# slp-rl/slamkit

Measured on NVIDIA H100. Metric: speech-tokens/sec (SLAM seq=1024), higher is better.
Workload: dtype bf16

## Files before the change

### slamkit_b200/csrc/gemm_tcgen05.cu

```cuda
#include "common.cuh"
#include <cudaTypedefs.h>
#include <stdio.h>
#include <mutex>
#include <type_traits>
#include <string.h>
#include <stdlib.h>
#include "kernels.h"
#include "../../include/slamkit_b200.h"

namespace {

constexpr int BM = 128;
constexpr int BK = 64;
constexpr int MMA_K = 16;
constexpr int GEMM_THREADS = 288;


struct GemmParams {
  int M, N, K;
  int batch;
  int a_mode;
  int passes;
  void* C;
  void* C_lo;
  int ldc;
  const void* bias;
  int bias_f32;
  const bf16* residual;
  const bf16* residual_lo;
  int ldr;
  int tiles_m, tiles_n;
  int out_f32;
  int round_before_res;
  int act;
  int col_gin, col_gout;
  int splits;
  float* splitk_ws;
  int tma_store;
  int reg_epi;
  int pdl;
  int sk_units;
  int sk_groups;
  int sk_G;
  int sk_colunits;
  int sk_carry;
  int units, n_groups;
  float* sk_ws;
  uint32_t* sk_flags;
  int epi;
  const bf16* aux;
  int ld_aux;
  const bf16* rope_cos;
  const bf16* rope_sin;
  const int* rope_pos;
  int rope_T, rope_cols, rope_maxpos, rope_rot;
};

template <int BN, int EW = 4>
struct GemmCfg {
  static constexpr int A_BYTES = BM * BK * 2;
  static constexpr int B_ATOMS = (BN + 63) / 64;
  static constexpr int B_BYTES = B_ATOMS * 64 * BK * 2;
  static constexpr int STAGE_BYTES = A_BYTES + B_BYTES;
  static constexpr int STAGES = (BN > 128) ? 4 : (BN > 64 ? 6 : 8);
  static constexpr int STAGING_BYTES = 4 * 2 * 4096;
  static constexpr int BAR_BYTES = 256;
  static constexpr int SMEM_BYTES = STAGES * STAGE_BYTES + STAGING_BYTES + BAR_BYTES + 1024;
  static_assert(BN % 64 == 0 || (BN == 224 && EW == 4), "a 32-column tail chunk only on the 224-wide tile");
  static_assert(STAGES * STAGE_BYTES >= BM * BN * 4, "the parked fp32 accumulator must fit in the stage ring");
  static_assert(SMEM_BYTES <= 227 * 1024, "sm_90 allows 227 KB of shared memory per block");
};

template <int BN>
SK_DEVINL uint32_t acc_chunk_addr(uint32_t base, int row, int chunk) {
  return base + (uint32_t)row * (BN * 4) + (uint32_t)((chunk ^ (row & 7)) << 4);
}
template <int BN>
SK_DEVINL void acc_park(uint32_t base, const float (&d)[BN / 2], int wg, int warp_in_wg, int lane) {
  const int r0 = 64 * wg + 16 * warp_in_wg + (lane >> 2);
#pragma unroll
  for (int j = 0; j < BN / 8; ++j) {
    const int chunk = 2 * j + ((lane & 3) >> 1);
    const uint32_t off = (uint32_t)(lane & 1) * 8u;
    asm volatile("st.shared.v2.f32 [%0], {%1, %2};" ::"r"(acc_chunk_addr<BN>(base, r0, chunk) + off), "f"(d[4 * j]),
                 "f"(d[4 * j + 1]) : "memory");
    asm volatile("st.shared.v2.f32 [%0], {%1, %2};" ::"r"(acc_chunk_addr<BN>(base, r0 + 8, chunk) + off), "f"(d[4 * j + 2]),
                 "f"(d[4 * j + 3]) : "memory");
  }
}
template <int BN>
SK_DEVINL void acc_ld_32x32(uint32_t base, uint32_t ta, uint32_t (&r)[32]) {
  const int row = (int)(ta >> 16) + (int)(threadIdx.x & 31);
  const int c0 = (int)(ta & 0xffffu) >> 2;
#pragma unroll
  for (int i = 0; i < 8; ++i)
    asm volatile("ld.shared.v4.b32 {%0, %1, %2, %3}, [%4];"
                 : "=r"(r[4 * i]), "=r"(r[4 * i + 1]), "=r"(r[4 * i + 2]), "=r"(r[4 * i + 3])
                 : "r"(acc_chunk_addr<BN>(base, row, c0 + i)) : "memory");
}

SK_DEVINL uint32_t staging_addr(uint32_t sbuf, int lane, int j, bool tail) {
  return tail ? sbuf + (uint32_t)lane * 64u + (uint32_t)((j ^ ((lane >> 1) & 3)) << 4)
              : sbuf + (uint32_t)lane * 128u + (uint32_t)((j ^ (lane & 7)) << 4);
}

SK_DEVINL float gelu_erf(float y) {
  const float a = fabsf(y);
  float t;
  asm("rcp.approx.ftz.f32 %0, %1;" : "=f"(t) : "f"(fmaf(0.3275911f * 0.70710678118654752440f, a, 1.0f)));
  float s = fmaf(0.5f * 1.061405429f, t, 0.5f * -1.453152027f);
  s = fmaf(s, t, 0.5f * 1.421413741f);
  s = fmaf(s, t, 0.5f * -0.284496736f);
  s = fmaf(s, t, 0.5f * 0.254829592f);
  const float e = ex2_approx((y * y) * -0.72134752044448170368f);
  return fmaf(-a, (s * t) * e, fmaxf(y, 0.0f));
}

SK_DEVINL float gelu_exact(float x) { return x * 0.5f * (1.0f + erff(x * 0.70710678118654752440f)); }
SK_DEVINL float gelu_exact_grad(float x) {
  const float cdf = 0.5f * (1.0f + erff(x * 0.70710678118654752440f));
  const float pdf = expf(-0.5f * x * x) * 0.39894228040143267794f;
  return cdf + x * pdf;
}

SK_DEVINL void stmatrix_x4(uint32_t addr, uint32_t a, uint32_t b, uint32_t c, uint32_t d) {
  asm volatile("stmatrix.sync.aligned.m8n8.x4.shared.b16 [%0], {%1, %2, %3, %4};" ::"r"(addr), "r"(a), "r"(b), "r"(c),
               "r"(d) : "memory");
}

template <bool SK>
struct WorkIter {
  int num_kb, splits, kb_per_split, total_items, tiles_n;
  int G, colunits, carry, units, n_groups, sk_groups, grp, mem;
  long sk_total, sk_cur, sk_end;
  int next_unit, next_item;
  int tile, split, kb_begin, kb_end, role;
  long unit_end_it;
  SK_DEVINL WorkIter(const GemmParams& p, int num_kb_, int kb_per_split_, int total_items_) {
    num_kb = num_kb_;
    splits = p.splits;
    kb_per_split = kb_per_split_;
    total_items = total_items_;
    tiles_n = p.tiles_n;
    G = p.sk_G;
    colunits = p.sk_colunits;
    carry = p.sk_carry;
    units = p.units;
    n_groups = p.n_groups;
    sk_groups = p.sk_groups;
    tile = split = kb_begin = kb_end = role = 0;
    unit_end_it = 0;
    sk_total = sk_cur = sk_end = 0;
    next_item = (int)blockIdx.x;
    next_unit = 0;
    grp = mem = 0;
    if (SK && p.sk_units > 0) {
      grp = (int)blockIdx.x / G;
      mem = (int)blockIdx.x - grp * G;
      next_item = total_items;
      next_unit = grp < n_groups ? p.sk_units + grp : units;
      if (grp < sk_groups) {
        sk_total = (long)p.sk_units * num_kb;
        sk_cur = sk_total * grp / sk_groups;
        sk_end = sk_total * (grp + 1) / sk_groups;
      }
    }
  }
  SK_DEVINL int tile_of(int unit) const { return colunits ? mem * tiles_n + unit : unit * G + mem; }
  SK_DEVINL bool next() {
    if (SK && sk_cur < sk_end && carry) {
      const int unit = (int)((sk_end - 1) / num_kb);
      const long ustart = (long)unit * num_kb;
      const long b = sk_cur > ustart ? sk_cur : ustart;
      kb_begin = (int)(b - ustart);
      kb_end = (int)(sk_end - ustart);
// ... 86 lines not shown
    const uint32_t aw[4] = {av.x, av.y, av.z, av.w};
#pragma unroll
    for (int i = 0; i < 4; ++i) {
      const float2 f = unpack_bf16(aw[i]);
      v[2 * i] = bf16_round(bf16_round(v[2 * i]) + f.x);
      v[2 * i + 1] = bf16_round(bf16_round(v[2 * i + 1]) + f.y);
    }
  }
  if (!p.residual) return;
  const uint4 rv = *reinterpret_cast<const uint4*>(p.residual + row * p.ldr + ocol);
  const uint32_t rw[4] = {rv.x, rv.y, rv.z, rv.w};
#pragma unroll
  for (int i = 0; i < 4; ++i) {
    const float2 f = unpack_bf16(rw[i]);
    if (p.round_before_res) {
      v[2 * i] = bf16_round(v[2 * i]) + f.x;
      v[2 * i + 1] = bf16_round(v[2 * i + 1]) + f.y;
    } else {
      v[2 * i] += f.x;
      v[2 * i + 1] += f.y;
    }
  }
  if (p.residual_lo) {
    const uint4 lv = *reinterpret_cast<const uint4*>(p.residual_lo + row * p.ldr + ocol);
    const uint32_t lw[4] = {lv.x, lv.y, lv.z, lv.w};
#pragma unroll
    for (int i = 0; i < 4; ++i) {
      const float2 f = unpack_bf16(lw[i]);
      v[2 * i] += f.x;
      v[2 * i + 1] += f.y;
    }
  }
}

constexpr int SK_SLOT_FLOATS = BM * 256;
SK_DEVINL size_t sk_slot_off(int chunk, int j4, int row_in_tile) { return ((size_t)(chunk * 8 + j4) * BM + row_in_tile) * 4; }

SK_DEVINL void sk_fixup_add(uint32_t (&r)[32], const float* ws, int chunk, int row_in_tile, int first_cta, int G, int n) {
  for (int c0 = 0; c0 < n; ++c0) {
    const float* slot = ws + (size_t)(first_cta + c0 * G) * SK_SLOT_FLOATS;
    float4 a[8];
#pragma unroll
    for (int j = 0; j < 8; ++j) a[j] = __ldcg(reinterpret_cast<const float4*>(slot + sk_slot_off(chunk, j, row_in_tile)));
#pragma unroll
    for (int j = 0; j < 8; ++j) {
      r[4 * j + 0] = __float_as_uint(__uint_as_float(r[4 * j + 0]) + a[j].x);
      r[4 * j + 1] = __float_as_uint(__uint_as_float(r[4 * j + 1]) + a[j].y);
      r[4 * j + 2] = __float_as_uint(__uint_as_float(r[4 * j + 2]) + a[j].z);
      r[4 * j + 3] = __float_as_uint(__uint_as_float(r[4 * j + 3]) + a[j].w);
    }
  }
}

template <int BN, bool A_MN, bool B_MN, bool SK, int EW>
__global__ void __launch_bounds__(GEMM_THREADS, 1)
gemm_wgmma_kernel(const __grid_constant__ CUtensorMap tmA, const __grid_constant__ CUtensorMap tmB,
                  const __grid_constant__ CUtensorMap tmA_lo, const __grid_constant__ CUtensorMap tmB_lo,
                  const __grid_constant__ CUtensorMap tmC, const __grid_constant__ CUtensorMap tmAux, GemmParams p) {
  using Cfg = GemmCfg<BN, EW>;
  static_assert(EW == 4 || (EW == 8 && BN == 256 && !SK), "8 epilogue warps: plain 256-wide tiles only");
  constexpr int CS = EW / 4;
  constexpr int NC64 = BN / 64;
  constexpr bool TAIL = BN % 64 != 0;
  griddep_launch();
  extern __shared__ uint8_t smem_raw[];
  const uint32_t smem_base = (smem_u32(smem_raw) + 1023u) & ~1023u;
  const uint32_t staging_base = smem_base + Cfg::STAGES * Cfg::STAGE_BYTES;
  const uint32_t bar_base = staging_base + Cfg::STAGING_BYTES;
  auto full_bar = [&](int s) { return bar_base + 8u * s; };
  auto empty_bar = [&](int s) { return bar_base + 8u * (Cfg::STAGES + s); };
  const uint32_t acc_free = bar_base + 8u * (2 * Cfg::STAGES);

  const int warp = threadIdx.x >> 5;
  const int lane = threadIdx.x & 31;
  const int tiles_per_batch = p.tiles_m * p.tiles_n;
  const int total_items = tiles_per_batch * p.batch * p.splits;
  const int num_kb_total = (p.K + BK - 1) / BK;
  const int kb_per_split = (num_kb_total + p.splits - 1) / p.splits;
  constexpr uint32_t STAGE_TX = Cfg::A_BYTES + (B_MN ? Cfg::B_ATOMS * 64 * BK * 2 : BN * BK * 2);

  if (threadIdx.x == 0) {
    tma_prefetch_desc(&tmA);
    tma_prefetch_desc(&tmB);
    for (int s = 0; s < Cfg::STAGES; ++s) {
      mbar_init(full_bar(s), 1);
      mbar_init(empty_bar(s), 8);
    }
    mbar_init(acc_free, 1);
    fence_mbar_init();
  }
  __syncthreads();
  griddep_wait();

  if (warp == 8) {
    if (lane == 0) {
      const bool split = p.passes == 3;
      const int n_stage = split ? Cfg::STAGES / 2 : Cfg::STAGES;
      const uint32_t stage_bytes = split ? 2u * Cfg::STAGE_BYTES : (uint32_t)Cfg::STAGE_BYTES;
      int stage = 0;
      uint32_t phase = 0;
      uint32_t acc_phase = 0;
      bool first = true;
      WorkIter<SK> w(p, num_kb_total, kb_per_split, total_items);
      while (w.next()) {
        if (!first && !p.reg_epi) {
          mbar_wait_nocall(acc_free, acc_phase);
          acc_phase ^= 1u;
        }
        first = false;
        const int bidx = w.tile / tiles_per_batch;
        const int r = w.tile - bidx * tiles_per_batch;
        const int m0 = (r / p.tiles_n) * BM;
        const int n_blk = r % p.tiles_n;
        const int n0 = n_blk * BN;
        for (int kb = w.kb_begin; kb < w.kb_end; ++kb) {
          mbar_wait_nocall(empty_bar(stage), phase ^ 1u);
          const uint32_t fb = full_bar(stage);
          mbar_arrive_expect_tx(fb, split ? 2u * STAGE_TX : STAGE_TX);
          for (int part = 0; part < (split ? 2 : 1); ++part) {
            const CUtensorMap* mapA = part ? &tmA_lo : &tmA;
            const CUtensorMap* mapB = part ? &tmB_lo : &tmB;
            const uint32_t sA = smem_base + stage * stage_bytes + part * Cfg::STAGE_BYTES;
            const uint32_t sB = sA + Cfg::A_BYTES;
            if (!A_MN) {
              if (p.a_mode & 2) {
                if (p.a_mode & 1) tma_load_3d(sA, mapA, fb, n_blk * 64, m0 + kb, bidx);
                else tma_load_3d(sA, mapA, fb, kb * BK, m0, bidx);
              } else {
                tma_load_2d(sA, mapA, fb, kb * BK, m0);
              }
            } else {
#pragma unroll
              for (int j = 0; j < BM / 64; ++j) tma_load_2d(sA + j * (BK * 128), mapA, fb, m0 + 64 * j, kb * BK);
            }
            if (!B_MN) {
              tma_load_2d(sB, mapB, fb, kb * BK, n0);
            } else {
#pragma unroll
              for (int j = 0; j < Cfg::B_ATOMS; ++j) tma_load_2d(sB + j * (BK * 128), mapB, fb, n0 + 64 * j, kb * BK);
            }
          }
          if (++stage == n_stage) { stage = 0; phase ^= 1u; }
        }
      }
    }
  } else {
    const int wg = warp >> 2;
    const int q = warp & 3;
    const int chalf = warp >> 2;
    const bool epi_warp = warp < EW;
    auto acc_ld = [&](uint32_t ta, uint32_t (&r)[32]) { acc_ld_32x32<BN>(smem_base, ta, r); };
    const bool split = p.passes == 3;
    const int n_stage = split ? Cfg::STAGES / 2 : Cfg::STAGES;
    const uint32_t stage_bytes = split ? 2u * Cfg::STAGE_BYTES : (uint32_t)Cfg::STAGE_BYTES;
    int stage = 0;
    uint32_t phase = 0;
    uint32_t store_cnt = 0;
    auto release_acc = [&] {
      fence_proxy_async();
      named_bar_sync(1, 256);
      if (threadIdx.x == 0) mbar_arrive(acc_free);
    };
    WorkIter<SK> w(p, num_kb_total, kb_per_split, total_items);
    while (w.next()) {
      {
        auto reg_epilogue = [&](const float (&acc)[BN / 2]) {
          const int rr = w.tile;
          const int m0 = (rr / p.tiles_n) * BM, n0 = (rr % p.tiles_n) * BN;
          const int row0 = m0 + 16 * warp;
          const uint32_t stg = staging_base + (uint32_t)warp * 4096u;
          auto emit = [&](const uint32_t (&pk)[16], const CUtensorMap* map, int col, bool tail) {
            const uint32_t sbuf = stg + (store_cnt & 1u) * 2048u;
            if (lane == 0) tma_store_wait_read<1>();
            __syncwarp();
            const int srow = (lane & 7) + (lane & 8);
#pragma unroll
            for (int jj = 0; jj < (tail ? 4 : 8); jj += 2) {
              const int ch = jj + (lane >> 4);
              const uint32_t addr = tail ? sbuf + (uint32_t)srow * 64u + (uint32_t)((ch ^ ((srow >> 1) & 3)) << 4)
                                         : sbuf + (uint32_t)srow * 128u + (uint32_t)((ch ^ (srow & 7)) << 4);
              stmatrix_x4(addr, pk[2 * jj], pk[2 * jj + 1], pk[2 * jj + 2], pk[2 * jj + 3]);
            }
            fence_proxy_async();
            __syncwarp();
            if (lane == 0) {
              tma_store_2d(map, sbuf, col, row0);
              tma_store_commit();
            }
            ++store_cnt;
          };
          auto pair_bf16 = [&](int j, int h) { return pack_bf16(acc[4 * j + 2 * h], acc[4 * j + 2 * h + 1]); };
          if (p.epi == 1) {
            if constexpr (BN == 256) {
#pragma unroll
              for (int i = 0; i < 2; ++i) {
                uint32_t pk[16];
#pragma unroll
                for (int t = 0; t < 16; ++t) pk[t] = pair_bf16(8 * i + (t >> 1), t & 1);
                emit(pk, &tmC, n0 + 64 * i, false);
#pragma unroll
                for (int t = 0; t < 16; ++t) pk[t] = pair_bf16(16 + 8 * i + (t >> 1), t & 1);
                emit(pk, &tmC, n0 + 128 + 64 * i, false);
#pragma unroll
                for (int t = 0; t < 16; ++t) {
                  const float2 gf = unpack_bf16(pair_bf16(8 * i + (t >> 1), t & 1));
                  const float2 uf = unpack_bf16(pair_bf16(16 + 8 * i + (t >> 1), t & 1));
                  const float2 sb = unpack_bf16(pack_bf16(silu_f(gf.x), silu_f(gf.y)));
                  pk[t] = pack_bf16(sb.x * uf.x, sb.y * uf.y);
                }
                emit(pk, &tmAux, (n0 >> 1) + 64 * i, false);
              }
            }
          } else {
#pragma unroll
            for (int c2 = 0; c2 < (BN + 63) / 64; ++c2) {
              const bool tail = BN % 64 != 0 && c2 == BN / 64;
              if (n0 + 64 * c2 >= p.N) continue;
              uint32_t pk[16];
#pragma unroll
              for (int t = 0; t < (tail ? 8 : 16); ++t) pk[t] = pair_bf16(8 * c2 + (t >> 1), t & 1);
              emit(pk, tail ? &tmAux : &tmC, n0 + 64 * c2, tail);
            }
          }
        };
        auto mainloop_park = [&](float (&acc)[BN / 2]) {
          const int k_iters = max(0, w.kb_end - w.kb_begin);
          int prev = -1;
          for (int kb = 0; kb < k_iters; ++kb) {
            mbar_wait_nocall(full_bar(stage), phase);
            wgmma_fence();
            const uint32_t s_hi = smem_base + stage * stage_bytes;
            for (int g = 0; g < (split ? 3 : 1); ++g) {
              const uint32_t sA = s_hi + (g == 2 ? Cfg::STAGE_BYTES : 0) + (uint32_t)wg * 8192u;
              const uint32_t sB = s_hi + Cfg::A_BYTES + (g == 1 ? Cfg::STAGE_BYTES : 0);
#pragma unroll
              for (int k = 0; k < BK / MMA_K; ++k) {
                const uint64_t adesc = A_MN ? gmma_desc_sw128(sA + k * (MMA_K * 128), BK * 128, 1024)
                                            : gmma_desc_sw128(sA + k * (MMA_K * 2), 16, 1024);
                const uint64_t bdesc = B_MN ? gmma_desc_sw128(sB + k * (MMA_K * 128), BK * 128, 1024)
                                            : gmma_desc_sw128(sB + k * (MMA_K * 2), 16, 1024);
                wgmma_bf16<BN, A_MN ? 1 : 0, B_MN ? 1 : 0>(acc, adesc, bdesc);
              }
            }
            wgmma_commit();
            wgmma_wait<1>();
            if (prev >= 0 && lane == 0) mbar_arrive(empty_bar(prev));
            prev = stage;
            if (++stage == n_stage) { stage = 0; phase ^= 1u; }
          }
          wgmma_wait<0>();
          if (prev >= 0 && lane == 0) mbar_arrive(empty_bar(prev));
          if constexpr (!SK && EW == 4) {
            if (p.reg_epi) {
              reg_epilogue(acc);
              return;
            }
          }
          named_bar_sync(1, 256);
          acc_park<BN>(smem_base, acc, wg, warp & 3, lane);
          named_bar_sync(1, 256);
        };
        if (SK && w.role == 3) {
          float acc[BN / 2];
          const int src = (int)blockIdx.x - w.G;
          if (threadIdx.x == 0) {
            for (int qq = 0; qq < 4; ++qq) {
              const uint32_t* f = p.sk_flags + src * 4 + qq;
              const uint64_t t0 = globaltimer_ns();
              while (ld_acquire_u32(f) == 0u) {
                __nanosleep(64);
                if (globaltimer_ns() - t0 > 8000000000ull) __trap();
              }
            }
            for (int qq = 0; qq < 4; ++qq) p.sk_flags[src * 4 + qq] = 0u;
          }
          named_bar_sync(1, 256);
          const float* slot = p.sk_ws + (size_t)src * SK_SLOT_FLOATS;
          const int r0 = 64 * wg + 16 * (warp & 3) + (lane >> 2);
#pragma unroll
          for (int j = 0; j < BN / 8; ++j) {
            const int col = 8 * j + 2 * (lane & 3);
#pragma unroll
            for (int h = 0; h < 2; ++h) {
              const float2 v = __ldcg(reinterpret_cast<const float2*>(slot + sk_slot_off(col >> 5, (col & 31) >> 2, r0 + 8 * h) +
                                                                      (col & 3)));
              acc[4 * j + 2 * h] = v.x;
              acc[4 * j + 2 * h + 1] = v.y;
            }
          }
          mainloop_park(acc);
        } else {
          float acc[BN / 2];
#pragma unroll
          for (int i = 0; i < BN / 2; ++i) acc[i] = 0.f;
          mainloop_park(acc);
        }
      }
      if (!SK && p.reg_epi) continue;
      if (!epi_warp) {
        release_acc();
        continue;
      }
      const int split_idx = w.split;
      const int bidx = w.tile / tiles_per_batch;
      const int rr = w.tile - bidx * tiles_per_batch;
      const int m0 = (rr / p.tiles_n) * BM;
      const int n0 = (rr % p.tiles_n) * BN;
      if (!SK && p.tma_store && p.epi == 2) {
        const int lpiece = lane & 7, lrsub = lane >> 3;
        const uint32_t sX = staging_base + (uint32_t)warp * (EW == 4 ? 8192u : 4096u);
        constexpr int NCH = BN / 64 / CS;
        const int c_lo = chalf * NCH;
        auto piece_off = [&](int bidx, int m0, int n0, int c2, size_t ld) -> size_t {
          const int acol = n0 + c2 * 64;
          const int gcol = (acol >> 7) * 256 + (acol & 127) + lpiece * 8;
          return (((size_t)bidx * p.M + m0 + q * 32 + lrsub) * ld + gcol) * sizeof(bf16);
        };
        const size_t row4_in = (size_t)4 * p.ld_aux * sizeof(bf16), row4_out = (size_t)4 * p.ldc * sizeof(bf16);
        uint4 gv[8], uv[8];
        auto gu_load_k = [&](int k, const uint8_t* base, int m0, int n0, int c2) {
          const int rin = m0 + q * 32 + 4 * k + lrsub;
          if (rin < p.M && n0 + c2 * 64 < p.N) {
            gv[k] = ldg128(base + k * row4_in);
            uv[k] = ldg128(base + k * row4_in + 256);
          } else {
            gv[k] = make_uint4(0u, 0u, 0u, 0u);
            uv[k] = make_uint4(0u, 0u, 0u, 0u);
          }
        };
        {
          const uint8_t* base = reinterpret_cast<const uint8_t*>(p.aux) + piece_off(bidx, m0, n0, c_lo, (size_t)p.ld_aux);
#pragma unroll
          for (int k = 0; k < 8; ++k) gu_load_k(k, base, m0, n0, c_lo);
        }
        const uint32_t taddr = (uint32_t)(q * 32) << 16;
#pragma unroll 1
        for (int c2 = c_lo; c2 < c_lo + NCH; ++c2) {
          const bool col_ok = n0 + c2 * 64 < p.N;
          {
            uint32_t r0[32], r1[32];
            acc_ld(taddr + c2 * 64, r0);
            acc_ld(taddr + c2 * 64 + 32, r1);
#pragma unroll
            for (int j = 0; j < 8; ++j) {
              const uint32_t* r = j < 4 ? r0 + 8 * j : r1 + 8 * (j - 4);
              const uint32_t dst = sX + (uint32_t)lane * 128u + (uint32_t)((j ^ (lane & 7)) << 4);
              asm volatile("st.shared.v4.b32 [%0], {%1, %2, %3, %4};" ::"r"(dst),
                           "r"(pack_bf16(__uint_as_float(r[0]), __uint_as_float(r[1]))),
                           "r"(pack_bf16(__uint_as_float(r[2]), __uint_as_float(r[3]))),
                           "r"(pack_bf16(__uint_as_float(r[4]), __uint_as_float(r[5]))),
                           "r"(pack_bf16(__uint_as_float(r[6]), __uint_as_float(r[7])))
                           : "memory");
            }
          }
          __syncwarp();
          const bool refill = c2 + 1 < c_lo + NCH;
          const int fm0 = m0, fn0 = n0, fc2 = c2 + 1;
          const uint8_t* fbase = reinterpret_cast<const uint8_t*>(p.aux) + piece_off(bidx, fm0, fn0, fc2, (size_t)p.ld_aux);
          uint8_t* obase = reinterpret_cast<uint8_t*>(p.C) + piece_off(bidx, m0, n0, c2, (size_t)p.ldc);
#pragma unroll
          for (int k = 0; k < 8; ++k) {
            const int rr2 = 4 * k + lrsub;
            const uint32_t off = (uint32_t)rr2 * 128u + (uint32_t)((lpiece ^ (rr2 & 7)) << 4);
            uint32_t dw[4];
            asm volatile("ld.shared.v4.b32 {%0, %1, %2, %3}, [%4];" : "=r"(dw[0]), "=r"(dw[1]), "=r"(dw[2]), "=r"(dw[3]) : "r"(sX + off));
            const uint32_t gw[4] = {gv[k].x, gv[k].y, gv[k].z, gv[k].w}, uw[4] = {uv[k].x, uv[k].y, uv[k].z, uv[k].w};
            if (refill) gu_load_k(k, fbase, fm0, fn0, fc2);
            uint32_t og[4], ou[4];
#pragma unroll
            for (int e = 0; e < 4; ++e) {
              const float2 gf = unpack_bf16(gw[e]);
              const float s0 = sigmoid_f(gf.x), s1 = sigmoid_f(gf.y);
              const uint32_t sil2 = pack_bf16(gf.x * s0, gf.y * s1);
              const float ds0 = s0 * (1.0f + gf.x * (1.0f - s0)), ds1 = s1 * (1.0f + gf.y * (1.0f - s1));
              const bf162 d2 = *reinterpret_cast<const bf162*>(&dw[e]);
              bf162 du2 = __hmul2(d2, *reinterpret_cast<const bf162*>(&uw[e]));
              bf162 o2 = __hmul2(d2, *reinterpret_cast<const bf162*>(&sil2));
              const float2 duf = __bfloat1622float2(du2);
              og[e] = pack_bf16(duf.x * ds0, duf.y * ds1);
              ou[e] = *reinterpret_cast<uint32_t*>(&o2);
            }
            if (col_ok && m0 + q * 32 + rr2 < p.M) {
              stg128(obase + k * row4_out, make_uint4(og[0], og[1], og[2], og[3]));
              stg128(obase + k * row4_out + 256, make_uint4(ou[0], ou[1], ou[2], ou[3]));
            }
          }
          __syncwarp();
        }
        release_acc();
        continue;
      }
      const int row_in_tile = q * 32 + lane;
      const int row_in = m0 + row_in_tile;
      const bool row_ok = row_in < p.M;
      const size_t row = (size_t)bidx * p.M + row_in;
      const uint32_t taddr = (uint32_t)(q * 32) << 16;
      const int first_contrib = (int)blockIdx.x + w.G;
      const int n_contrib = (SK && w.role == 2) ? w.n_contrib() : 0;
      if (SK && w.role == 1) {
        float* slot = p.sk_ws + (size_t)blockIdx.x * SK_SLOT_FLOATS;
#pragma unroll 1
        for (int c = 0; c < BN / 32; ++c) {
          uint32_t r[32];
          acc_ld(taddr + c * 32, r);
#pragma unroll
          for (int j = 0; j < 8; ++j)
            __stcg(reinterpret_cast<float4*>(slot + sk_slot_off(c, j, row_in_tile)),
                   make_float4(__uint_as_float(r[4 * j]), __uint_as_float(r[4 * j + 1]), __uint_as_float(r[4 * j + 2]),
                               __uint_as_float(r[4 * j + 3])));
        }
        __threadfence();
        __syncwarp();
        if (lane == 0) st_release_u32(p.sk_flags + blockIdx.x * 4 + q, 1u);
      } else {
        if (SK && w.role == 2) {
          if (lane == 0) {
            for (int i = 0; i < n_contrib; ++i) {
              const int c = first_contrib + i * w.G;
              const uint32_t* f = p.sk_flags + c * 4 + q;
              const uint64_t t0 = globaltimer_ns();
              while (ld_acquire_u32(f) == 0u) {
                __nanosleep(64);
                if (globaltimer_ns() - t0 > 8000000000ull) __trap();
              }
            }
          }
          __syncwarp();
        }
        auto stage_store = [&](const CUtensorMap* map, const uint32_t (&pk)[32], int col, auto tail_c) {
          constexpr bool tail = decltype(tail_c)::value;
          const uint32_t sbuf = staging_base + (EW == 4 ? (uint32_t)warp * 8192u + (store_cnt & 1u) * 4096u : (uint32_t)warp * 4096u);
          if (lane == 0) {
            if constexpr (EW == 4) tma_store_wait_read<1>(); else tma_store_wait_read<0>();
          }
// ... 427 lines not shown
PFN_cuTensorMapEncodeTiled_v12000 g_encode = nullptr;
std::once_flag g_encode_once;

void load_encode() {
  void* fn = nullptr;
  cudaDriverEntryPointQueryResult qres;
  cudaError_t e = cudaGetDriverEntryPoint("cuTensorMapEncodeTiled", &fn, cudaEnableDefault, &qres);
  if (e == cudaSuccess && qres == cudaDriverEntryPointSuccess) g_encode = (PFN_cuTensorMapEncodeTiled_v12000)fn;
}

}

int sk_make_tmap_2d(CUtensorMap* out, const void* ptr, int elem_bytes, uint64_t inner, uint64_t outer, uint64_t ld,
                    uint32_t box_inner, uint32_t box_outer) {
  std::call_once(g_encode_once, load_encode);
  SK_REQUIRE(g_encode != nullptr, "cuTensorMapEncodeTiled driver entry point not available");
  SK_REQUIRE((reinterpret_cast<uintptr_t>(ptr) & 15) == 0, "TMA base pointer must be 16-byte aligned");
  SK_REQUIRE((ld * elem_bytes) % 16 == 0, "TMA row pitch must be a multiple of 16 bytes (ld=%llu)",
             (unsigned long long)ld);
  SK_REQUIRE(box_inner * elem_bytes == 128 || box_inner * elem_bytes == 64, "box inner extent must be 128 (or 64) bytes");
  cuuint64_t dims[2] = {inner, outer};
  cuuint64_t strides[1] = {ld * (uint64_t)elem_bytes};
  cuuint32_t box[2] = {box_inner, box_outer};
  cuuint32_t estr[2] = {1, 1};
  CUtensorMapDataType dt = elem_bytes == 2 ? CU_TENSOR_MAP_DATA_TYPE_BFLOAT16 : CU_TENSOR_MAP_DATA_TYPE_FLOAT32;
  CUresult r = g_encode(out, dt, 2, const_cast<void*>(ptr), dims, strides, box, estr, CU_TENSOR_MAP_INTERLEAVE_NONE,
                        box_inner * elem_bytes == 64 ? CU_TENSOR_MAP_SWIZZLE_64B : CU_TENSOR_MAP_SWIZZLE_128B,
                        CU_TENSOR_MAP_L2_PROMOTION_L2_256B,
                        CU_TENSOR_MAP_FLOAT_OOB_FILL_NONE);
  SK_REQUIRE(r == CUDA_SUCCESS, "cuTensorMapEncodeTiled failed with CUresult %d (inner=%llu outer=%llu ld=%llu)", (int)r,
             (unsigned long long)inner, (unsigned long long)outer, (unsigned long long)ld);
  return 0;
}

int sk_make_tmap_3d(CUtensorMap* out, const void* ptr, uint64_t inner, uint64_t rows, uint64_t batch, uint64_t row_stride,
                    uint64_t batch_stride, uint32_t box_rows) {
  std::call_once(g_encode_once, load_encode);
  SK_REQUIRE(g_encode != nullptr, "cuTensorMapEncodeTiled driver entry point not available");
  SK_REQUIRE((reinterpret_cast<uintptr_t>(ptr) & 15) == 0, "TMA base pointer must be 16-byte aligned");
  SK_REQUIRE((row_stride * 2) % 16 == 0 && (batch_stride * 2) % 16 == 0, "TMA strides must be multiples of 16 bytes");
  cuuint64_t dims[3] = {inner, rows, batch};
  cuuint64_t strides[2] = {row_stride * 2, batch_stride * 2};
  cuuint32_t box[3] = {64, box_rows, 1};
  cuuint32_t estr[3] = {1, 1, 1};
  CUresult r = g_encode(out, CU_TENSOR_MAP_DATA_TYPE_BFLOAT16, 3, const_cast<void*>(ptr), dims, strides, box, estr,
                        CU_TENSOR_MAP_INTERLEAVE_NONE, CU_TENSOR_MAP_SWIZZLE_128B, CU_TENSOR_MAP_L2_PROMOTION_L2_256B,
                        CU_TENSOR_MAP_FLOAT_OOB_FILL_NONE);
  SK_REQUIRE(r == CUDA_SUCCESS, "cuTensorMapEncodeTiled(3d) failed with CUresult %d", (int)r);
  return 0;
}

namespace {

template <int BN, bool A_MN, bool B_MN, bool SK, int EW = 4>
int launch_gemm(const CUtensorMap* tm, const GemmParams& p, int grid, cudaStream_t stream) {
  using Cfg = GemmCfg<BN, EW>;
  static bool attr_set = false;
  if (!attr_set) {
    SK_CUDA_CHECK(cudaFuncSetAttribute(gemm_wgmma_kernel<BN, A_MN, B_MN, SK, EW>, cudaFuncAttributeMaxDynamicSharedMemorySize,
                                       Cfg::SMEM_BYTES));
    attr_set = true;
  }
  sk_prof_begin(0, stream);
  cudaError_t lerr = sk_launch_pdl_if(p.pdl != 0, gemm_wgmma_kernel<BN, A_MN, B_MN, SK, EW>, dim3(grid), dim3(GEMM_THREADS), (size_t)Cfg::SMEM_BYTES, stream,
                                   tm[0], tm[1], tm[2], tm[3], tm[4], tm[5], p);
  sk_prof_end(stream);
  SK_CUDA_CHECK(lerr);
  SK_LAUNCH_CHECK();
  return 0;
}

template <int BN, bool SK, int EW = 4>
int dispatch_major(bool a_mn, bool b_mn, const CUtensorMap* tm, const GemmParams& p, int grid, cudaStream_t s) {
  if (!a_mn && !b_mn) return launch_gemm<BN, false, false, SK, EW>(tm, p, grid, s);
  if (!a_mn && b_mn) return launch_gemm<BN, false, true, SK, EW>(tm, p, grid, s);
  if (a_mn && !b_mn) return launch_gemm<BN, true, false, SK, EW>(tm, p, grid, s);
  return launch_gemm<BN, true, true, SK, EW>(tm, p, grid, s);
}

inline int tile_cost(int bn) { return bn >= 256 ? 100 : (bn > 128 ? 61 + (bn - 128) * 39 / 128 : (bn == 128 ? 61 : 54)); }

constexpr size_t SK_FLAG_BYTES = 4096;

}

size_t sk_gemm_ws_min_bytes(void) { return (size_t)sk_num_sms() * SK_SLOT_FLOATS * sizeof(float) + SK_FLAG_BYTES; }

int sk_pick_bn(int M, int N, int force_bn, bool fit_forced, bool fit, bool whole_heads) {
  if (force_bn == 64 || force_bn == 128 || force_bn == 256) return force_bn;
  if (fit_forced && (force_bn == 192 || (force_bn == 224 && !whole_heads))) return force_bn;
  const int nsm = sk_num_sms();
  auto cost = [&](int bn) {
    const long tiles = (long)((M + BM - 1) / BM) * ((N + bn - 1) / bn);
    return ((tiles + nsm - 1) / nsm) * tile_cost(bn);
  };
  int best = 256;
  long best_cost = cost(256);
  for (const int bn : {128, 64}) {
    if (cost(bn) * 100 < best_cost * 75) {
      best_cost = cost(bn);
      best = bn;
    }
  }
  if (best == 256 && fit && N % 256 != 0) {
    for (const int bn : {224, 192}) {
      if (!(whole_heads && bn % 64 != 0) && cost(bn) * 100 < best_cost * 95) {
        best_cost = cost(bn);
        best = bn;
      }
    }
  }
  return best;
}

namespace {

int plan_gemm(const SkGemmEx& g, GemmParams& p, int& BN, int& ew, int& grid) {
// ... 95 lines not shown
      SK_REQUIRE(BN == 256 && g.N % 256 == 0 && g.aux_out && g.ld_aux_out % 8 == 0 && !g.bias,
                 "gemm: SwiGLU-forward epilogue needs N = 2F with F %% 128 == 0 and an act output");
    } else if (g.epi == 2) {
      SK_REQUIRE(BN == 256 && g.N % 128 == 0 && g.aux && g.ld_aux % 8 == 0 && !g.bias,
                 "gemm: SwiGLU-backward epilogue needs N = F with F %% 128 == 0 and the saved gu activation");
    } else if (g.epi == 3) {
      SK_REQUIRE(g.rope_cos && g.rope_sin && g.rope_T > 0 && g.rope_maxpos > 0 && g.rope_cols % 64 == 0 && g.N % 64 == 0 &&
                     !g.bias_f32,
                 "gemm: RoPE epilogue needs cos/sin tables, 64-column heads and a bf16 bias");
      SK_REQUIRE(p.rope_rot == 16 || p.rope_rot == 32 || p.rope_rot == 64,
                 "gemm: RoPE epilogue rotary width rope_rot=%d is not supported (16, 32 or 64)", g.rope_rot);
    } else if (g.epi == 4) {
      SK_REQUIRE(BN % 64 == 0 && g.N % 64 == 0 && g.aux_out && g.ld_aux_out >= g.N && g.ld_aux_out % 8 == 0 && !g.bias_f32 &&
                     (reinterpret_cast<uintptr_t>(g.aux_out) & 15) == 0,
                 "gemm: GELU-forward epilogue needs N %% 64 == 0, an act output (pitch >= N) and a bf16 bias");
    } else if (g.epi == 5) {
      SK_REQUIRE(BN % 64 == 0 && g.N % 64 == 0 && g.aux && g.ld_aux >= g.N && g.ld_aux % 8 == 0 && !g.bias &&
                     (reinterpret_cast<uintptr_t>(g.aux) & 15) == 0,
                 "gemm: GELU-backward epilogue needs N %% 64 == 0, the saved pre-activation (pitch >= N) and no bias");
    } else {
      SK_REQUIRE(false, "gemm: unknown fused epilogue %d", g.epi);
    }
  }
  p.sk_G = 1;
  if (sk_ok && BN == 256 && p.splits == 1 && num_kb >= sk_min_kb && (p.tiles_n <= 8 || p.tiles_m <= 8)) {
    const int colunits = p.tiles_n <= 8 ? 0 : 1;
    const int G = colunits ? p.tiles_m : p.tiles_n;
    const int units = colunits ? p.tiles_n : p.tiles_m;
    const int n_groups = nsm / G;
    const int rem = units % n_groups;
    const long slots = ((long)(units + n_groups - 1) / n_groups) * n_groups;
    const bool multiwave = units > n_groups;
    if (n_groups >= 1 && rem != 0 && (slots - units) * 100 >= slots * sk_min_idle &&
        (!colunits || multiwave || sk_env >= 2)) {
      if (colunits && multiwave) {
        p.sk_units = rem + n_groups;
        p.sk_groups = n_groups;
        p.sk_carry = 1;
      } else {
        p.sk_units = rem;
        p.sk_groups = n_groups < rem * sk_ranges ? n_groups : rem * sk_ranges;
      }
      p.sk_G = G;
      p.sk_colunits = colunits;
      p.units = units;
      p.n_groups = n_groups;
      p.sk_ws = reinterpret_cast<float*>(g.splitk_ws);
      p.sk_flags = reinterpret_cast<uint32_t*>(reinterpret_cast<uint8_t*>(g.splitk_ws) + ws_data_bytes);
    }
  }
  const long work = tiles * p.splits;
  grid = p.sk_units > 0 ? p.n_groups * p.sk_G : (int)(work < nsm ? work : nsm);
  static const int ew_env = [] { const char* e = getenv("SK_GEMM_EW"); return e ? atoi(e) : 0; }();
  ew = (p.sk_units == 0 && BN == 256 && p.tma_store && (ew_env == 8 || (ew_env == 0 && (g.epi == 2 || g.epi == 3 || g.epi == 4 || g.epi == 5)))) ? 8 : 4;
  p.reg_epi = (p.tma_store && p.sk_units == 0 && ew == 4 && !g.bias && !g.act && !g.residual && (g.epi == 0 || g.epi == 1)) ? 1 : 0;
  return 0;
}

}

int sk_gemm_plan_ex(const SkGemmEx& g, SkGemmPlan* out) {
  GemmParams p;
  int BN = 0, ew = 0, grid = 0;
  const int rc = plan_gemm(g, p, BN, ew, grid);
  if (rc) return rc;
  out->bn = BN;
  out->epi_warps = ew;
  out->splits = p.splits;
  out->sk_units = p.sk_units;
  out->sk_groups = p.sk_groups;
  out->sk_G = p.sk_G;
  out->sk_colunits = p.sk_colunits;
  out->tma_store = p.tma_store;
  out->grid = grid;
  return 0;
}

int sk_gemm_ex_launch(const SkGemmEx& g, cudaStream_t stream) {
  GemmParams p;
  int BN = 0, ew = 0, grid = 0;
  const int rc0 = plan_gemm(g, p, BN, ew, grid);
  if (rc0) return rc0;
  const bool use3d = g.a_rows > 0;
  CUtensorMap tm[6];
  const void* As[2] = {g.A, g.passes == 3 ? g.A_lo : g.A};
  const void* Bs[2] = {g.B, g.passes == 3 ? g.B_lo : g.B};
  for (int i = 0; i < 2; ++i) {
    int rc;
    CUtensorMap* ta = &tm[i == 0 ? 0 : 2];
    CUtensorMap* tb = &tm[i == 0 ? 1 : 3];
    if (use3d) {
      rc = sk_make_tmap_3d(ta, As[i], (uint64_t)g.a_inner, (uint64_t)g.a_rows, (uint64_t)g.batch, (uint64_t)g.a_row_stride,
                           (uint64_t)g.a_batch_stride, BM);
    } else if (!g.a_mn) {
      rc = sk_make_tmap_2d(ta, As[i], 2, (uint64_t)g.K, (uint64_t)g.M, (uint64_t)g.lda, BK, BM);
    } else {
      rc = sk_make_tmap_2d(ta, As[i], 2, (uint64_t)g.M, (uint64_t)g.K, (uint64_t)g.lda, 64, BK);
    }
    if (rc) return rc;
    if (!g.b_mn) rc = sk_make_tmap_2d(tb, Bs[i], 2, (uint64_t)g.K, (uint64_t)g.N, (uint64_t)g.ldb, BK, (uint32_t)BN);
    else         rc = sk_make_tmap_2d(tb, Bs[i], 2, (uint64_t)g.N, (uint64_t)g.K, (uint64_t)g.ldb, 64, BK);
    if (rc) return rc;
  }
  tm[4] = tm[0];
  const uint32_t box_rows = p.reg_epi ? 16 : 32;
  if (p.tma_store) {
    const int rc2 = sk_make_tmap_2d(&tm[4], g.C, 2, (uint64_t)(g.epi == 2 ? 2 * g.N : g.N), (uint64_t)g.M, (uint64_t)g.ldc, 64, box_rows);
    if (rc2) return rc2;
  }
  tm[5] = tm[4];
  if (g.epi == 1) {
    const int rc3 = sk_make_tmap_2d(&tm[5], g.aux_out, 2, (uint64_t)g.N / 2, (uint64_t)g.M, (uint64_t)g.ld_aux_out, 64, box_rows);
    if (rc3) return rc3;
  } else if (g.epi == 4) {
    const int rc3 = sk_make_tmap_2d(&tm[5], g.aux_out, 2, (uint64_t)g.N, (uint64_t)g.M, (uint64_t)g.ld_aux_out, 64, 32);
    if (rc3) return rc3;
  } else if (p.tma_store && BN % 64 != 0) {
    const int rc3 = sk_make_tmap_2d(&tm[5], g.C, 2, (uint64_t)g.N, (uint64_t)g.M, (uint64_t)g.ldc, 32, box_rows);
    if (rc3) return rc3;
  }
  int rc;
  if (p.sk_units > 0) {
    rc = dispatch_major<256, true>(g.a_mn, g.b_mn, tm, p, grid, stream);
  } else if (ew == 8) {
    rc = dispatch_major<256, false, 8>(g.a_mn, g.b_mn, tm, p, grid, stream);
  } else {
    switch (BN) {
      case 256: rc = dispatch_major<256, false>(g.a_mn, g.b_mn, tm, p, grid, stream); break;
      case 224: rc = dispatch_major<224, false>(g.a_mn, g.b_mn, tm, p, grid, stream); break;
      case 192: rc = dispatch_major<192, false>(g.a_mn, g.b_mn, tm, p, grid, stream); break;
      case 128: rc = dispatch_major<128, false>(g.a_mn, g.b_mn, tm, p, grid, stream); break;
      default:  rc = dispatch_major<64, false>(g.a_mn, g.b_mn, tm, p, grid, stream); break;
    }
  }
  if (rc) return rc;
  if (p.splits > 1) {
    SK_REQUIRE(g.residual == nullptr || g.residual == g.C, "gemm: split-K supports only in-place accumulation");
    const long n8 = (long)g.M * g.N / 8;
    int blocks = (int)((n8 + 255) / 256);
    if (blocks > sk_num_sms() * 8) blocks = sk_num_sms() * 8;
    sk_prof_begin(0, stream);
    SK_CUDA_CHECK(sk_launch_pdl(splitk_reduce_kernel, dim3(blocks), dim3(256), (size_t)(0), stream, p.splitk_ws, reinterpret_cast<bf16*>(g.C), g.M, g.N, g.ldc, p.splits,
                                                     g.residual != nullptr, g.round_before_res));
    sk_prof_end(stream);
    SK_LAUNCH_CHECK();
  }
  return 0;
}

SkGemmEx sk_gemm_desc(int M, int N, int K, const void* A, int lda, int a_mn, const void* B, int ldb, int b_mn, void* C,
                      int ldc, int out_f32, const void* bias, const void* residual, int ldr, int round_before_res, int act,
                      int force_bn, void* splitk_ws, size_t splitk_ws_bytes) {
  SkGemmEx g;
  memset(&g, 0, sizeof(g));
  g.M = M; g.N = N; g.K = K; g.batch = 1; g.passes = 1;
  g.A = A; g.lda = lda; g.a_mn = a_mn;
  g.B = B; g.ldb = ldb; g.b_mn = b_mn;
  g.C = C; g.ldc = ldc; g.out_f32 = out_f32;
  g.bias = bias; g.residual = residual; g.ldr = ldr; g.round_before_res = round_before_res; g.act = act;
  g.force_bn = force_bn;
  g.pdl = 1;
  g.splitk_ws = splitk_ws;
  g.splitk_ws_bytes = splitk_ws_bytes;
  return g;
}
int sk_gemm_launch(int M, int N, int K, const void* A, int lda, int a_mn, const void* B, int ldb, int b_mn, void* C,
                   int ldc, int out_f32, const void* bias, const void* residual, int ldr, int round_before_res, int act,
                   int force_bn, cudaStream_t stream, void* splitk_ws, size_t splitk_ws_bytes) {
  return sk_gemm_ex_launch(sk_gemm_desc(M, N, K, A, lda, a_mn, B, ldb, b_mn, C, ldc, out_f32, bias, residual, ldr,
                                        round_before_res, act, force_bn, splitk_ws, splitk_ws_bytes),
                           stream);
}

int sk_linear_swiglu_fwd_launch(int M, int F, int K, const void* x, const void* Wgu, void* gu, void* act, cudaStream_t s) {
  SkGemmEx g;
// ... 61 lines not shown
```

Baseline: 165,800.

## Fuse SwiGLU backward into register epilogue with TMA-prefetched gate/up operands

Adds a GU kernel variant for the epi==2 (SwiGLU backward) GEMM. The accumulator is combined in registers with gate/up operands that TMA double-buffers into per-warp shared memory, and the results go out through TMA stores, replacing the parked-accumulator shared-memory epilogue. It also adds a register epilogue with residual add for narrower tiles, and stops epi==2 from using 8 epilogue warps. The GU variant drops to 3 pipeline stages to make room for operand buffers, which may reduce mainloop latency hiding.

```diff
diff --git a/slamkit_b200/csrc/gemm_tcgen05.cu b/slamkit_b200/csrc/gemm_tcgen05.cu
--- a/slamkit_b200/csrc/gemm_tcgen05.cu
+++ b/slamkit_b200/csrc/gemm_tcgen05.cu
@@ -56,16 +56,17 @@
   int rope_T, rope_cols, rope_maxpos, rope_rot;
 };
 
-template <int BN, int EW = 4>
+template <int BN, int EW = 4, bool GU = false>
 struct GemmCfg {
   static constexpr int A_BYTES = BM * BK * 2;
   static constexpr int B_ATOMS = (BN + 63) / 64;
   static constexpr int B_BYTES = B_ATOMS * 64 * BK * 2;
   static constexpr int STAGE_BYTES = A_BYTES + B_BYTES;
-  static constexpr int STAGES = (BN > 128) ? 4 : (BN > 64 ? 6 : 8);
-  static constexpr int STAGING_BYTES = 4 * 2 * 4096;
+  static constexpr int STAGES = GU ? 3 : ((BN > 128) ? 4 : (BN > 64 ? 6 : 8));
+  static constexpr int STAGING_BYTES = GU ? 8 * 2048 : 4 * 2 * 4096;
+  static constexpr int OPND_BYTES = GU ? 8 * 2 * 4096 : 0;
   static constexpr int BAR_BYTES = 256;
-  static constexpr int SMEM_BYTES = STAGES * STAGE_BYTES + STAGING_BYTES + BAR_BYTES + 1024;
+  static constexpr int SMEM_BYTES = STAGES * STAGE_BYTES + STAGING_BYTES + OPND_BYTES + BAR_BYTES + 1024;
   static_assert(BN % 64 == 0 || (BN == 224 && EW == 4), "a 32-column tail chunk only on the 224-wide tile");
   static_assert(STAGES * STAGE_BYTES >= BM * BN * 4, "the parked fp32 accumulator must fit in the stage ring");
   static_assert(SMEM_BYTES <= 227 * 1024, "sm_90 allows 227 KB of shared memory per block");
@@ -121,6 +122,24 @@
   const float cdf = 0.5f * (1.0f + erff(x * 0.70710678118654752440f));
   const float pdf = expf(-0.5f * x * x) * 0.39894228040143267794f;
   return cdf + x * pdf;
+}
+
+SK_DEVINL void swiglu_bwd_pair(uint32_t d, uint32_t g, uint32_t u, uint32_t& og, uint32_t& ou) {
+  const float2 gf = unpack_bf16(g);
+  const float s0 = sigmoid_f(gf.x), s1 = sigmoid_f(gf.y);
+  const uint32_t sil2 = pack_bf16(gf.x * s0, gf.y * s1);
+  const float ds0 = s0 * (1.0f + gf.x * (1.0f - s0)), ds1 = s1 * (1.0f + gf.y * (1.0f - s1));
+  const bf162 d2 = *reinterpret_cast<const bf162*>(&d);
+  const bf162 du2 = __hmul2(d2, *reinterpret_cast<const bf162*>(&u));
+  bf162 o2 = __hmul2(d2, *reinterpret_cast<const bf162*>(&sil2));
+  const float2 duf = __bfloat1622float2(du2);
+  og = pack_bf16(duf.x * ds0, duf.y * ds1);
+  ou = *reinterpret_cast<uint32_t*>(&o2);
+}
+
+SK_DEVINL void ldmatrix_x4(uint32_t addr, uint32_t& a, uint32_t& b, uint32_t& c, uint32_t& d) {
+  asm volatile("ldmatrix.sync.aligned.m8n8.x4.shared.b16 {%0, %1, %2, %3}, [%4];"
+               : "=r"(a), "=r"(b), "=r"(c), "=r"(d) : "r"(addr) : "memory");
 }
 
 SK_DEVINL void stmatrix_x4(uint32_t addr, uint32_t a, uint32_t b, uint32_t c, uint32_t d) {
@@ -313,13 +332,14 @@
   }
 }
 
-template <int BN, bool A_MN, bool B_MN, bool SK, int EW>
+template <int BN, bool A_MN, bool B_MN, bool SK, int EW, bool GU = false>
 __global__ void __launch_bounds__(GEMM_THREADS, 1)
 gemm_wgmma_kernel(const __grid_constant__ CUtensorMap tmA, const __grid_constant__ CUtensorMap tmB,
                   const __grid_constant__ CUtensorMap tmA_lo, const __grid_constant__ CUtensorMap tmB_lo,
                   const __grid_constant__ CUtensorMap tmC, const __grid_constant__ CUtensorMap tmAux, GemmParams p) {
-  using Cfg = GemmCfg<BN, EW>;
+  using Cfg = GemmCfg<BN, EW, GU>;
   static_assert(EW == 4 || (EW == 8 && BN == 256 && !SK), "8 epilogue warps: plain 256-wide tiles only");
+  static_assert(!GU || (BN == 256 && EW == 4 && !SK), "the SwiGLU-backward register epilogue runs on plain 256-wide tiles");
   constexpr int CS = EW / 4;
   constexpr int NC64 = BN / 64;
   constexpr bool TAIL = BN % 64 != 0;
@@ -327,10 +347,12 @@
   extern __shared__ uint8_t smem_raw[];
   const uint32_t smem_base = (smem_u32(smem_raw) + 1023u) & ~1023u;
   const uint32_t staging_base = smem_base + Cfg::STAGES * Cfg::STAGE_BYTES;
-  const uint32_t bar_base = staging_base + Cfg::STAGING_BYTES;
+  const uint32_t opnd_base = staging_base + Cfg::STAGING_BYTES;
+  const uint32_t bar_base = opnd_base + Cfg::OPND_BYTES;
   auto full_bar = [&](int s) { return bar_base + 8u * s; };
   auto empty_bar = [&](int s) { return bar_base + 8u * (Cfg::STAGES + s); };
   const uint32_t acc_free = bar_base + 8u * (2 * Cfg::STAGES);
+  auto opnd_bar = [&](int w, int b) { return bar_base + 8u * (2 * Cfg::STAGES + 1 + 2 * w + b); };
 
   const int warp = threadIdx.x >> 5;
   const int lane = threadIdx.x & 31;
@@ -348,6 +370,8 @@
       mbar_init(empty_bar(s), 8);
     }
     mbar_init(acc_free, 1);
+    if constexpr (GU)
+      for (int i = 0; i < 16; ++i) mbar_init(opnd_bar(i >> 1, i & 1), 1);
     fence_mbar_init();
   }
   __syncthreads();
@@ -355,6 +379,7 @@
 
   if (warp == 8) {
     if (lane == 0) {
+      if constexpr (GU) tma_prefetch_desc(&tmAux);
       const bool split = p.passes == 3;
       const int n_stage = split ? Cfg::STAGES / 2 : Cfg::STAGES;
       const uint32_t stage_bytes = split ? 2u * Cfg::STAGE_BYTES : (uint32_t)Cfg::STAGE_BYTES;
@@ -417,12 +442,25 @@
     int stage = 0;
     uint32_t phase = 0;
     uint32_t store_cnt = 0;
+    uint32_t opnd_phase = 0;
     auto release_acc = [&] {
       fence_proxy_async();
       named_bar_sync(1, 256);
       if (threadIdx.x == 0) mbar_arrive(acc_free);
     };
     WorkIter<SK> w(p, num_kb_total, kb_per_split, total_items);
+    auto opnd_load = [&](int c2) {
+      const int rr = w.tile;
+      const int m0 = (rr / p.tiles_n) * BM, acol = (rr % p.tiles_n) * BN + 64 * c2;
+      if (lane == 0 && acol < p.N) {
+        const uint32_t buf = opnd_base + (uint32_t)warp * 8192u + (uint32_t)(c2 & 1) * 4096u;
+        const int g0 = (acol >> 7) * 256 + (acol & 127);
+        fence_proxy_async();
+        mbar_arrive_expect_tx(opnd_bar(warp, c2 & 1), 4096u);
+        tma_load_2d(buf, &tmAux, opnd_bar(warp, c2 & 1), g0, m0 + 16 * warp);
+        tma_load_2d(buf + 2048u, &tmAux, opnd_bar(warp, c2 & 1), g0 + 128, m0 + 16 * warp);
+      }
+    };
     while (w.next()) {
       {
         auto reg_epilogue = [&](const float (&acc)[BN / 2]) {
@@ -431,8 +469,10 @@
           const int row0 = m0 + 16 * warp;
           const uint32_t stg = staging_base + (uint32_t)warp * 4096u;
           auto emit = [&](const uint32_t (&pk)[16], const CUtensorMap* map, int col, bool tail) {
-            const uint32_t sbuf = stg + (store_cnt & 1u) * 2048u;
-            if (lane == 0) tma_store_wait_read<1>();
+            const uint32_t sbuf = GU ? staging_base + (uint32_t)warp * 2048u : stg + (store_cnt & 1u) * 2048u;
+            if (lane == 0) {
+              if constexpr (GU) tma_store_wait_read<0>(); else tma_store_wait_read<1>();
+            }
             __syncwarp();
             const int srow = (lane & 7) + (lane & 8);
 #pragma unroll
@@ -451,7 +491,36 @@
             ++store_cnt;
           };
           auto pair_bf16 = [&](int j, int h) { return pack_bf16(acc[4 * j + 2 * h], acc[4 * j + 2 * h + 1]); };
-          if (p.epi == 1) {
+          if constexpr (GU) {
+            uint32_t dpk[BN / 4];
+#pragma unroll
+            for (int t = 0; t < BN / 4; ++t) dpk[t] = pair_bf16(t >> 1, t & 1);
+            const int srow = (lane & 7) + (lane & 8);
+#pragma unroll
+            for (int c2 = 0; c2 < 4; ++c2) {
+              const int acol = n0 + 64 * c2;
+              if (acol >= p.N) break;
+              const uint32_t buf = opnd_base + (uint32_t)warp * 8192u + (uint32_t)(c2 & 1) * 4096u;
+              mbar_wait_nocall(opnd_bar(warp, c2 & 1), (opnd_phase >> (c2 & 1)) & 1u);
+              opnd_phase ^= 1u << (c2 & 1);
+              uint32_t gk[16], uk[16];
+#pragma unroll
+              for (int jj = 0; jj < 8; jj += 2) {
+                const int ch = jj + (lane >> 4);
+                const uint32_t off = (uint32_t)srow * 128u + (uint32_t)((ch ^ (srow & 7)) << 4);
+                ldmatrix_x4(buf + off, gk[2 * jj], gk[2 * jj + 1], gk[2 * jj + 2], gk[2 * jj + 3]);
+                ldmatrix_x4(buf + 2048u + off, uk[2 * jj], uk[2 * jj + 1], uk[2 * jj + 2], uk[2 * jj + 3]);
+              }
+              __syncwarp();
+              if (c2 + 2 < 4) opnd_load(c2 + 2);
+              uint32_t og[16], ou[16];
+#pragma unroll
+              for (int t = 0; t < 16; ++t) swiglu_bwd_pair(dpk[16 * c2 + t], gk[t], uk[t], og[t], ou[t]);
+              const int g0 = (acol >> 7) * 256 + (acol & 127);
+              emit(og, &tmC, g0, false);
+              emit(ou, &tmC, g0 + 128, false);
+            }
+          } else if (p.epi == 1) {
             if constexpr (BN == 256) {
 #pragma unroll
               for (int i = 0; i < 2; ++i) {
@@ -471,6 +540,38 @@
                 }
                 emit(pk, &tmAux, (n0 >> 1) + 64 * i, false);
               }
+            }
+          } else if (BN < 256 && p.residual) {
+            const int rowa = row0 + (lane >> 2);
+            auto res_ld = [&](int c2, uint32_t (&rv)[16]) {
+#pragma unroll
+              for (int t = 0; t < 16; ++t) {
+                const int row = rowa + 8 * (t & 1), col = n0 + 64 * c2 + 8 * (t >> 1);
+                rv[t] = (row < p.M && col < p.N && (BN % 64 == 0 || c2 < BN / 64 || t < 8))
+                            ? __ldg(reinterpret_cast<const uint32_t*>(p.residual + (size_t)row * p.ldr + col + 2 * (lane & 3)))
+                            : 0u;
+              }
+            };
+            uint32_t rv[2][16];
+            res_ld(0, rv[0]);
+#pragma unroll
+            for (int c2 = 0; c2 < (BN + 63) / 64; ++c2) {
+              const bool tail = BN % 64 != 0 && c2 == BN / 64;
+              if (n0 + 64 * c2 >= p.N) break;
+              if (c2 + 1 < (BN + 63) / 64) res_ld(c2 + 1, rv[(c2 + 1) & 1]);
+              uint32_t pk[16];
+#pragma unroll
+              for (int t = 0; t < (tail ? 8 : 16); ++t) {
+                const int j = 8 * c2 + (t >> 1), h = t & 1;
+                float a0 = acc[4 * j + 2 * h], a1 = acc[4 * j + 2 * h + 1];
+                if (p.round_before_res) {
+                  const float2 r = unpack_bf16(pack_bf16(a0, a1));
+                  a0 = r.x; a1 = r.y;
+                }
+                const float2 f = unpack_bf16(rv[c2 & 1][t]);
+                pk[t] = pack_bf16(a0 + f.x, a1 + f.y);
+              }
+              emit(pk, tail ? &tmAux : &tmC, n0 + 64 * c2, tail);
             }
           } else {
 #pragma unroll
@@ -511,7 +612,10 @@
           }
           wgmma_wait<0>();
           if (prev >= 0 && lane == 0) mbar_arrive(empty_bar(prev));
-          if constexpr (!SK && EW == 4) {
+          if constexpr (GU) {
+            reg_epilogue(acc);
+            return;
+          } else if constexpr (!SK && EW == 4) {
             if (p.reg_epi) {
               reg_epilogue(acc);
               return;
@@ -521,6 +625,10 @@
           acc_park<BN>(smem_base, acc, wg, warp & 3, lane);
           named_bar_sync(1, 256);
         };
+        if constexpr (GU) {
+          opnd_load(0);
+          opnd_load(1);
+        }
         if (SK && w.role == 3) {
           float acc[BN / 2];
           const int src = (int)blockIdx.x - w.G;
@@ -557,7 +665,7 @@
           mainloop_park(acc);
         }
       }
-      if (!SK && p.reg_epi) continue;
+      if (GU || (!SK && p.reg_epi)) continue;
       if (!epi_warp) {
         release_acc();
         continue;
@@ -629,18 +737,7 @@
             if (refill) gu_load_k(k, fbase, fm0, fn0, fc2);
             uint32_t og[4], ou[4];
 #pragma unroll
-            for (int e = 0; e < 4; ++e) {
-              const float2 gf = unpack_bf16(gw[e]);
-              const float s0 = sigmoid_f(gf.x), s1 = sigmoid_f(gf.y);
-              const uint32_t sil2 = pack_bf16(gf.x * s0, gf.y * s1);
-              const float ds0 = s0 * (1.0f + gf.x * (1.0f - s0)), ds1 = s1 * (1.0f + gf.y * (1.0f - s1));
-              const bf162 d2 = *reinterpret_cast<const bf162*>(&dw[e]);
-              bf162 du2 = __hmul2(d2, *reinterpret_cast<const bf162*>(&uw[e]));
-              bf162 o2 = __hmul2(d2, *reinterpret_cast<const bf162*>(&sil2));
-              const float2 duf = __bfloat1622float2(du2);
-              og[e] = pack_bf16(duf.x * ds0, duf.y * ds1);
-              ou[e] = *reinterpret_cast<uint32_t*>(&o2);
-            }
+            for (int e = 0; e < 4; ++e) swiglu_bwd_pair(dw[e], gw[e], uw[e], og[e], ou[e]);
             if (col_ok && m0 + q * 32 + rr2 < p.M) {
               stg128(obase + k * row4_out, make_uint4(og[0], og[1], og[2], og[3]));
               stg128(obase + k * row4_out + 256, make_uint4(ou[0], ou[1], ou[2], ou[3]));
@@ -1174,17 +1271,17 @@
 
 namespace {
 
-template <int BN, bool A_MN, bool B_MN, bool SK, int EW = 4>
+template <int BN, bool A_MN, bool B_MN, bool SK, int EW = 4, bool GU = false>
 int launch_gemm(const CUtensorMap* tm, const GemmParams& p, int grid, cudaStream_t stream) {
-  using Cfg = GemmCfg<BN, EW>;
+  using Cfg = GemmCfg<BN, EW, GU>;
   static bool attr_set = false;
   if (!attr_set) {
-    SK_CUDA_CHECK(cudaFuncSetAttribute(gemm_wgmma_kernel<BN, A_MN, B_MN, SK, EW>, cudaFuncAttributeMaxDynamicSharedMemorySize,
-                                       Cfg::SMEM_BYTES));
+    SK_CUDA_CHECK(cudaFuncSetAttribute(gemm_wgmma_kernel<BN, A_MN, B_MN, SK, EW, GU>,
+                                       cudaFuncAttributeMaxDynamicSharedMemorySize, Cfg::SMEM_BYTES));
     attr_set = true;
   }
   sk_prof_begin(0, stream);
-  cudaError_t lerr = sk_launch_pdl_if(p.pdl != 0, gemm_wgmma_kernel<BN, A_MN, B_MN, SK, EW>, dim3(grid), dim3(GEMM_THREADS), (size_t)Cfg::SMEM_BYTES, stream,
+  cudaError_t lerr = sk_launch_pdl_if(p.pdl != 0, gemm_wgmma_kernel<BN, A_MN, B_MN, SK, EW, GU>, dim3(grid), dim3(GEMM_THREADS), (size_t)Cfg::SMEM_BYTES, stream,
                                    tm[0], tm[1], tm[2], tm[3], tm[4], tm[5], p);
   sk_prof_end(stream);
   SK_CUDA_CHECK(lerr);
@@ -1386,8 +1483,10 @@
   const long work = tiles * p.splits;
   grid = p.sk_units > 0 ? p.n_groups * p.sk_G : (int)(work < nsm ? work : nsm);
   static const int ew_env = [] { const char* e = getenv("SK_GEMM_EW"); return e ? atoi(e) : 0; }();
-  ew = (p.sk_units == 0 && BN == 256 && p.tma_store && (ew_env == 8 || (ew_env == 0 && (g.epi == 2 || g.epi == 3 || g.epi == 4 || g.epi == 5)))) ? 8 : 4;
-  p.reg_epi = (p.tma_store && p.sk_units == 0 && ew == 4 && !g.bias && !g.act && !g.residual && (g.epi == 0 || g.epi == 1)) ? 1 : 0;
+  ew = (p.sk_units == 0 && BN == 256 && p.tma_store && (ew_env == 8 || (ew_env == 0 && (g.epi == 3 || g.epi == 4 || g.epi == 5)))) ? 8 : 4;
+  const bool reg_res = g.epi == 0 && g.residual != nullptr && g.residual != g.C && !g.residual_lo && BN < 256;
+  p.reg_epi = (p.tma_store && p.sk_units == 0 && ew == 4 && !g.bias && !g.act && (!g.residual || reg_res) &&
+               (g.epi == 0 || g.epi == 1 || (g.epi == 2 && !g.a_mn && g.b_mn))) ? 1 : 0;
   return 0;
 }
 
@@ -1449,12 +1548,17 @@
   } else if (g.epi == 4) {
     const int rc3 = sk_make_tmap_2d(&tm[5], g.aux_out, 2, (uint64_t)g.N, (uint64_t)g.M, (uint64_t)g.ld_aux_out, 64, 32);
     if (rc3) return rc3;
+  } else if (g.epi == 2 && p.reg_epi) {
+    const int rc3 = sk_make_tmap_2d(&tm[5], g.aux, 2, (uint64_t)(2 * g.N), (uint64_t)g.M, (uint64_t)g.ld_aux, 64, 16);
+    if (rc3) return rc3;
   } else if (p.tma_store && BN % 64 != 0) {
     const int rc3 = sk_make_tmap_2d(&tm[5], g.C, 2, (uint64_t)g.N, (uint64_t)g.M, (uint64_t)g.ldc, 32, box_rows);
     if (rc3) return rc3;
   }
   int rc;
-  if (p.sk_units > 0) {
+  if (g.epi == 2 && p.reg_epi) {
+    rc = launch_gemm<256, false, true, false, 4, true>(tm, p, grid, stream);
+  } else if (p.sk_units > 0) {
     rc = dispatch_major<256, true>(g.a_mn, g.b_mn, tm, p, grid, stream);
   } else if (ew == 8) {
     rc = dispatch_major<256, false, 8>(g.a_mn, g.b_mn, tm, p, grid, stream);
```

Result: faster. 169,000, median of 6 (+1.9%).
